# agentmorris/MegaDetector

Hardware: AMD Instinct MI355X
Metric: images/sec (whole node) MDv5a @1280px batch inference (higher is better)
Workload: dtype bf16

## Files before the change

megadetector_amd/csrc/conv_v2.cpp:

```cpp

#include <algorithm>
#include <type_traits>

#include "conv_device.h"

namespace mdhip {
namespace MDHIP_ST {

namespace {

constexpr int v2_lds_bytes(int bm, int bn) { return 2 * (bm + bn) * 128; }
constexpr int v2_ring_lds_bytes(int bm, int bn) { return (3 * bm + 2 * bn) * 128; }
constexpr int v2_blocks_per_cu(int bm, int bn, int nw) {
    int b = 163840 / v2_lds_bytes(bm, bn);
    if (b > 32 / nw) b = 32 / nw;
    if (b > 2) b = 2;
    return b < 1 ? 1 : b;
}
constexpr int v2_waves_per_simd(int bm, int bn, int nw) {
    int w = v2_blocks_per_cu(bm, bn, nw) * nw / 4;
    return w < 1 ? 1 : w;
}

}

template <int BM, int BN, int WM, int WN, int PROF = 0, bool UP = false, int PW = 0, int RA = 2, int DEC = 0>
__global__ void __launch_bounds__(WM * WN * 64, v2_waves_per_simd(BM, BN, WM * WN))
conv_v2_kernel(const ConvArgs p) {
#if defined(__HIP_DEVICE_COMPILE__)
    constexpr int NW = WM * WN;
    constexpr int TM = BM / WM, TN = BN / WN;
    constexpr int FM = TM / 16, FN = TN / 16;
    constexpr int A_BYTES = BM * 128, B_BYTES = BN * 128, STAGE = A_BYTES + B_BYTES;
    constexpr int B_INSTR = BN / 8;
    constexpr int A_PER = BM / 8 / NW, B_PER = (B_INSTR + NW - 1) / NW;
    constexpr bool B_RAGGED = (B_INSTR % NW) != 0;
    static_assert((BM / 8) % NW == 0, "the activation tile must split evenly over the waves");
    static_assert(RA == 2 || (RA == 3 && PW != 0 && !UP), "the three-stage activation ring is a pointwise instantiation");
    auto a_stage = [](int sa) __attribute__((always_inline)) { return RA == 2 ? sa * STAGE : sa * A_BYTES; };
    auto b_stage = [](int sb) __attribute__((always_inline)) { return RA == 2 ? sb * STAGE + A_BYTES : RA * A_BYTES + sb * B_BYTES; };
    static_assert(TM % 16 == 0 && TN % 16 == 0 && TM % 8 == 0, "wave tile must be a multiple of 16x16");

    extern __shared__ __attribute__((aligned(16))) char smem_generic[];
    lds_char* const smem = (lds_char*)smem_generic;

    const int tid = threadIdx.x;
    const int lane = tid & 63;
    const int wave = __builtin_amdgcn_readfirstlane(tid >> 6);
    const int wm = wave / WN, wn = wave % WN;

    const int xcd = blockIdx.x & 7, slot = blockIdx.x >> 3;
    const int tile_n = slot % p.tiles_n;
    const int ms = slot / p.tiles_n;
    const int xcd_first = xcd * p.tiles_per_xcd;
    const int xcd_tiles = min(p.tiles_per_xcd, p.tiles_m - xcd_first);
    const int my_tiles = (xcd_tiles > ms) ? (xcd_tiles - ms + p.m_streams - 1) / p.m_streams : 0;
    if (my_tiles <= 0) return;
    const int first_tile = xcd_first + ms;
    const int tile_step = p.m_streams;
    const int last_tile = first_tile + (my_tiles - 1) * tile_step;
    const int n0 = tile_n * BN;
    const int KT = p.k_pad >> 6;
    const int total_steps = my_tiles * KT;

    const int lr = lane >> 3;
    const int jj = (lane & 7) ^ lr;
    const __amdgpu_buffer_rsrc_t b_rsrc = __builtin_amdgcn_make_buffer_rsrc(
        (void*)(p.wgt + (size_t)n0 * p.k_pad), 0, kNumRecords, kRsrcFlags);
    unsigned b_off[B_PER];
#pragma unroll
    for (int i = 0; i < B_PER; ++i) {
        const int row = (i * NW + wave) * 8 + lr;
        b_off[i] = (n0 + row < p.n_rows) ? (unsigned)(row * p.k_pad + jj * 8) * 2u : kOOB;
    }

    __amdgpu_buffer_rsrc_t a_rsrc = b_rsrc;
    unsigned a_off[A_PER];
    uint32_t a_mask[A_PER];
    const int up_slabs = UP ? p.up_slabs : 0;
    [[maybe_unused]] const __amdgpu_buffer_rsrc_t u_rsrc = __builtin_amdgcn_make_buffer_rsrc((void*)(UP ? p.in_up : p.in), 0, kNumRecords, kRsrcFlags);
    [[maybe_unused]] unsigned u_off[UP ? A_PER : 1];
    int c8 = 0, ts = 0;
    uint32_t tapbit = 1;
    unsigned tapoff = 0;
    int l_kt = 0, l_tile = first_tile;
    bool l_live = true;
    [[maybe_unused]] int lb_kt = 0;
    const int kh = p.ntaps / p.kw;
    const unsigned wrap_c = (unsigned)(p.ld_in * 2 - p.C8 * 16);
    const unsigned wrap_r = (unsigned)((p.W - p.kw) * p.ld_in * 2);

    auto init_tile = [&](int tile_m) __attribute__((always_inline)) {
        if constexpr (PW) {
            const int m0 = tile_m * BM;
            const long long left = ((long long)p.M - m0) * p.ld_in * 2;
            a_rsrc = __builtin_amdgcn_make_buffer_rsrc((void*)(p.in + (long long)m0 * p.ld_in), 0,
                                                       (int)(left > 0x7fffffffLL ? 0x7fffffffLL : left), kRsrcFlags);
#pragma unroll
            for (int i = 0; i < A_PER; ++i) {
                const int row = (i * NW + wave) * 8 + lr;
                a_off[i] = (unsigned)(row * p.ld_in * 2 + jj * 16);
                a_mask[i] = 1u;
            }
            c8 = jj; ts = 0; tapbit = 1; tapoff = 0;
            return;
        }
        const int m0 = tile_m * BM;
        const int b0 = conv_udiv(m0, p.HoWo, p.rcp_howo);
        const int rem0 = m0 - b0 * p.HoWo;
        const int oy0 = conv_udiv(rem0, p.Wo, p.rcp_wo);
        const int ox0 = rem0 - oy0 * p.Wo;
        const long long base_px = (long long)(b0 * p.H + oy0 * p.stride - p.pad) * p.W + (ox0 * p.stride - p.pad);
        a_rsrc = __builtin_amdgcn_make_buffer_rsrc((void*)(p.in + base_px * p.ld_in), 0, kNumRecords, kRsrcFlags);
#pragma unroll
        for (int i = 0; i < A_PER; ++i) {
            const int row = (i * NW + wave) * 8 + lr;
            const int m = m0 + row;
            uint32_t mask = 0;
            unsigned off = 0;
            if (m < p.M) {
                const int b = conv_udiv(m, p.HoWo, p.rcp_howo);
                const int rem = m - b * p.HoWo;
                const int oy = conv_udiv(rem, p.Wo, p.rcp_wo);
                const int ox = rem - oy * p.Wo;
                const int iy0 = oy * p.stride - p.pad;
                const int ix0 = ox * p.stride - p.pad;
                const long long px = (long long)(b * p.H + iy0) * p.W + ix0;
                off = (unsigned)((px - base_px) * p.ld_in * 2);
                if constexpr (UP)
                    u_off[i] = (unsigned)((((long long)b * (p.H >> 1) + (oy >> 1)) * (p.W >> 1) + (ox >> 1)) * p.ld_up * 2 + jj * 16);
                uint32_t cols = 0, rows = 0;
#pragma unroll
                for (int t = 0; t < 3; ++t) {
                    cols |= (t < p.kw && (unsigned)(ix0 + t) < (unsigned)p.W) ? 1u << t : 0u;
                    rows |= (t < kh && (unsigned)(iy0 + t) < (unsigned)p.H) ? 1u << t : 0u;
                }
                mask = ((rows & 1u) ? cols : 0u) | ((rows & 2u) ? cols << p.kw : 0u) | ((rows & 4u) ? cols << (2 * p.kw) : 0u);
            }
            a_off[i] = off;
            a_mask[i] = mask;
        }
        c8 = jj; ts = 0; tapbit = 1; tapoff = (unsigned)jj * 16u;
    };

    [[maybe_unused]] const bool pw_tail_bad = (p.C8 & 7) != 0 && jj >= (p.C8 & 7);
    auto advance = [&]() __attribute__((always_inline)) {
        if (++l_kt == KT) {
            l_kt = 0;
            if (l_tile == last_tile) {
                l_live = false;
#pragma unroll
                for (int i = 0; i < A_PER; ++i) a_mask[i] = 0;
            } else {
                l_tile += tile_step;
                init_tile(l_tile);
            }
        } else {
            if constexpr (PW) {
                if constexpr (PW == 2) {
                    if (l_kt == KT - 1 && pw_tail_bad) {
#pragma unroll
                        for (int i = 0; i < A_PER; ++i) a_off[i] = kOOB;
                    }
                }
            }
            c8 += 8;
            tapoff += 128u;
            const bool w = c8 >= p.C8;
            c8 = w ? c8 - p.C8 : c8;
            tapoff += w ? wrap_c : 0u;
            tapbit = w ? tapbit << 1 : tapbit;
            ts += w ? 1 : 0;
            const bool w2 = ts == p.kw;
            ts = w2 ? 0 : ts;
            tapoff += w2 ? wrap_r : 0u;
        }
    };

    auto dma_a = [&](int buf, int i) __attribute__((always_inline)) {
        if constexpr ((PROF & 16) != 0) return;
        if constexpr (UP) {
            if (l_kt < up_slabs) {
                MDHIP_DMA16(u_rsrc, smem + buf * STAGE + (i * NW + wave) * 1024, (a_mask[i] & tapbit) ? u_off[i] : kOOB, l_kt * 128);
                return;
            }
        }
        if constexpr (PW) {
            MDHIP_DMA16(a_rsrc, smem + a_stage(buf) + (i * NW + wave) * 1024, a_off[i], l_kt * 128);
        } else {
            const unsigned voff = (a_mask[i] & tapbit) ? a_off[i] + tapoff : kOOB;
            MDHIP_DMA16(a_rsrc, smem + buf * STAGE + (i * NW + wave) * 1024, voff, 0);
        }
    };
    auto dma_b = [&](int buf, int i) __attribute__((always_inline)) {
        if constexpr ((PROF & 16) != 0) return;
        if (B_RAGGED && i == B_PER - 1 && wave >= B_INSTR % NW) return;
        const unsigned voff = (PW || l_live) ? b_off[i] : kOOB;
        MDHIP_DMA16(b_rsrc, smem + b_stage(buf) + (i * NW + wave) * 1024, voff, (RA == 3 ? lb_kt : l_kt) * 128);
    };

    const int frag_row_off = (lane & 15) * 128;
    const int frag_ch0 = (((lane >> 4) ^ (lane & 7)) * 16);
    const int a_frag_base = (wm * TM) * 128 + frag_row_off;
    const int b_frag_base = (wn * TN) * 128 + frag_row_off;
    auto read_x = [&](int buf, int kk, int i) -> frag8_t {
        if constexpr ((PROF & 32) != 0) return frag_dummy(lane + i);
        return *(const __attribute__((address_space(3))) frag8_t*)(smem + a_stage(buf) + a_frag_base + i * 2048 +
                                                                 (frag_ch0 ^ (kk * 64)));
    };
    auto read_w = [&](int buf, int kk, int j) -> frag8_t {
        if constexpr ((PROF & 32) != 0) return frag_dummy(lane + j);
        return *(const __attribute__((address_space(3))) frag8_t*)(smem + b_stage(buf) + b_frag_base + j * 2048 +
                                                                 (frag_ch0 ^ (kk * 64)));
    };

    f32x4 acc[FM][FN];
#pragma unroll
    for (int i = 0; i < FM; ++i)
#pragma unroll
        for (int j = 0; j < FN; ++j) acc[i][j] = f32x4{0.f, 0.f, 0.f, 0.f};

    const int q4 = lane >> 4;
    auto epilogue_t = [&](int tile_m, auto has_res_t, auto out_f32_t, auto out_f8_t) {
#pragma clang fp contract(off)
        constexpr bool HAS_RES = decltype(has_res_t)::value;
        constexpr bool OUT_F32 = decltype(out_f32_t)::value;
        constexpr bool OUT_F8 = decltype(out_f8_t)::value;
        const int m0 = tile_m * BM + wm * TM + (lane & 15);
        const int nbase = n0 + wn * TN + q4 * 4;
        int lane_e = lane;
        asm volatile("" : "+v"(lane_e));
        float neg_log2e = kNegLog2e;
        asm volatile("" : "+v"(neg_log2e));
        const int ml = wm * TM + (lane_e & 15);
        const int qe = lane_e >> 4;
        const int npair0 = n0 + wn * TN + qe * 8;
        const int nlast = n0 + wn * TN + (FN - 1) * 16 + qe * 4;
        const long long rows_left = (long long)p.M - (long long)tile_m * BM;
        const __amdgpu_buffer_rsrc_t o_rsrc = __builtin_amdgcn_make_buffer_rsrc(
            (void*)((uint16_t*)p.out + (size_t)tile_m * BM * p.ld_out), 0,
            (OUT_F32 || OUT_F8) ? 0 : (int)min(rows_left * p.ld_out * 2, 0x7fffffffLL), kRsrcFlags);
        const unsigned o_pair = ((unsigned)ml * (unsigned)p.ld_out + (unsigned)npair0) * 2u;
        const unsigned o_last = ((unsigned)ml * (unsigned)p.ld_out + (unsigned)nlast) * 2u;
        const unsigned o_step = 16u * (unsigned)p.ld_out * 2u;
        const __amdgpu_buffer_rsrc_t r_rsrc = __builtin_amdgcn_make_buffer_rsrc(
            (void*)(p.res + (HAS_RES ? (size_t)tile_m * BM * p.ld_res : 0)), 0,
            HAS_RES ? (int)min(rows_left * p.ld_res * 2, 0x7fffffffLL) : 0, kRsrcFlags);
        const unsigned r_col = ((unsigned)ml * (unsigned)p.ld_res + (unsigned)(n0 + wn * TN + qe * 4)) * 2u;
        const unsigned r_step = 16u * (unsigned)p.ld_res * 2u;
        float bv[FN][4];
#pragma unroll
        for (int j = 0; j < FN; ++j) {
            const int nb = n0 + wn * TN + j * 16;
            bv[j][0] = bv[j][1] = bv[j][2] = bv[j][3] = 0.f;
            if (nb < p.n_rows) {
                f32x16 b16;
                const unsigned long long ba = (unsigned long long)(p.bias + nb);
                const unsigned long long bs =
                    ((unsigned long long)(unsigned)__builtin_amdgcn_readfirstlane((int)(ba >> 32)) << 32) |
                    (unsigned)__builtin_amdgcn_readfirstlane((int)ba);
                asm volatile("s_load_dwordx16 %0, %1, 0x0\n\ts_waitcnt lgkmcnt(0)" : "=s"(b16) : "s"(bs) : "memory");
                const f32x4 g0 = {b16[0], b16[1], b16[2], b16[3]}, g1 = {b16[4], b16[5], b16[6], b16[7]},
                            g2 = {b16[8], b16[9], b16[10], b16[11]}, g3 = {b16[12], b16[13], b16[14], b16[15]};
                const f32x4 g = q4 == 0 ? g0 : (q4 == 1 ? g1 : (q4 == 2 ? g2 : g3));
                bv[j][0] = g[0]; bv[j][1] = g[1]; bv[j][2] = g[2]; bv[j][3] = g[3];
            }
        }
        uint2 rrow[2][FN];
        auto fetch_res_row = [&](int i, uint2 (&r)[FN]) {
#pragma unroll
            for (int j = 0; j < FN; ++j) {
                const u32x2 t = __builtin_amdgcn_raw_buffer_load_b64(r_rsrc, (int)(r_col + (unsigned)i * r_step + (unsigned)(j * 32)), 0, 0);
                r[j] = make_uint2(t[0], t[1]);
            }
        };
        if constexpr (HAS_RES) fetch_res_row(0, rrow[0]);
#pragma unroll
        for (int i = 0; i < FM; ++i) {
            if constexpr (HAS_RES) {
                if (i + 1 < FM) fetch_res_row(i + 1, rrow[(i + 1) & 1]);
            }
            const int m = m0 + i * 16;
            float v[FN][4];
#pragma unroll
            for (int j = 0; j < FN; ++j) {
#pragma unroll
                for (int r = 0; r < 4; r += 2) {
                    const mdhip_f32x2 t = mdhip_f32x2{acc[i][j][r], acc[i][j][r + 1]} + mdhip_f32x2{bv[j][r], bv[j][r + 1]};
                    v[j][r] = t[0];
                    v[j][r + 1] = t[1];
                }
                acc[i][j] = f32x4{0.f, 0.f, 0.f, 0.f};
            }
            if ((PROF & 4) == 0 && p.act) {
#pragma unroll
                for (int j = 0; j < FN; ++j) {
#pragma unroll
                    for (int r = 0; r < 4; r += 2) {
                        const mdhip_f32x2 t = silu_f32x2(mdhip_f32x2{v[j][r], v[j][r + 1]}, neg_log2e);
                        v[j][r] = t[0];
                        v[j][r + 1] = t[1];
                    }
                }
            }
#pragma unroll
            for (int j = 0; j < FN; ++j) {
                if constexpr (HAS_RES) {
                    const uint2 rv = rrow[i & 1][j];
                    v[j][0] += st_unpack((uint16_t)(rv.x & 0xffff));
                    v[j][1] += st_unpack((uint16_t)(rv.x >> 16));
                    v[j][2] += st_unpack((uint16_t)(rv.y & 0xffff));
                    v[j][3] += st_unpack((uint16_t)(rv.y >> 16));
                }
            }
            if constexpr ((PROF & 2) != 0) {
#pragma unroll
                for (int j = 0; j < FN; ++j) asm volatile("" ::"v"(v[j][0]), "v"(v[j][1]), "v"(v[j][2]), "v"(v[j][3]));
            } else if constexpr (OUT_F32 && DEC != 0) {
#pragma unroll
                for (int j = 0; j < FN; ++j) {
                    const int n = nbase + j * 16;
                    if (m < p.M && n < p.N) mdhip_decode_store(p, m, n, v[j]);
                }
            } else if constexpr (OUT_F32) {
#pragma unroll
                for (int j = 0; j < FN; ++j) {
                    const int n = nbase + j * 16;
                    if (m < p.M && n < p.N)
                        *(float4*)((float*)p.out + (size_t)m * p.ld_out + n) = make_float4(v[j][0], v[j][1], v[j][2], v[j][3]);
                }
            } else if constexpr (OUT_F8) {
                const __amdgpu_buffer_rsrc_t o8_rsrc = __builtin_amdgcn_make_buffer_rsrc(
                    (void*)((uint8_t*)p.out + (size_t)tile_m * BM * p.ld_out), 0, (int)min(rows_left * p.ld_out, 0x7fffffffLL), kRsrcFlags);
                const unsigned row8 = (unsigned)(ml + i * 16) * (unsigned)p.ld_out;
#pragma unroll
                for (int j = 0; j + 1 < FN; j += 2) {
                    const unsigned a0 = pack_e4m3x4(v[j][0], v[j][1], v[j][2], v[j][3], p.out_qscale);
                    const unsigned b0 = pack_e4m3x4(v[j + 1][0], v[j + 1][1], v[j + 1][2], v[j + 1][3], p.out_qscale);
                    const auto s0 = __builtin_amdgcn_permlane32_swap(a0, b0, false, false);
                    const auto t0 = __builtin_amdgcn_permlane16_swap(s0[0], s0[1], false, false);
                    const int n = npair0 + j * 16;
                    __builtin_amdgcn_raw_buffer_store_b64(u32x2{t0[0], t0[1]}, o8_rsrc, (int)(n < p.N ? row8 + (unsigned)n : kOOB), 0, 0);
                }
                if (FN & 1) {
                    const int j = FN - 1;
                    __builtin_amdgcn_raw_buffer_store_b32(pack_e4m3x4(v[j][0], v[j][1], v[j][2], v[j][3], p.out_qscale), o8_rsrc,
                                                          (int)(nlast < p.N ? row8 + (unsigned)nlast : kOOB), 0, 0);
                }
            } else {
#pragma unroll
                for (int j = 0; j + 1 < FN; j += 2) {
                    unsigned a0 = st_pack2(v[j][0], v[j][1]), a1 = st_pack2(v[j][2], v[j][3]);
                    unsigned b0 = st_pack2(v[j + 1][0], v[j + 1][1]), b1 = st_pack2(v[j + 1][2], v[j + 1][3]);
                    auto s0 = __builtin_amdgcn_permlane32_swap(a0, b0, false, false);
                    auto s1 = __builtin_amdgcn_permlane32_swap(a1, b1, false, false);
                    auto t0 = __builtin_amdgcn_permlane16_swap(s0[0], s0[1], false, false);
                    auto t1 = __builtin_amdgcn_permlane16_swap(s1[0], s1[1], false, false);
                    const unsigned off = o_pair + (unsigned)i * o_step + (unsigned)(j * 32);
                    __builtin_amdgcn_raw_buffer_store_b128(u32x4{t0[0], t1[0], t0[1], t1[1]}, o_rsrc,
                                                           (int)(npair0 + j * 16 < p.N ? off : kOOB), 0, 0);
                }
                if (FN & 1) {
                    const int j = FN - 1;
                    __builtin_amdgcn_raw_buffer_store_b64(u32x2{st_pack2(v[j][0], v[j][1]), st_pack2(v[j][2], v[j][3])}, o_rsrc,
                                                          (int)(nlast < p.N ? o_last + (unsigned)i * o_step : kOOB), 0, 0);
                }
            }
        }
    };
    auto epilogue = [&](int tile_m) {
        if constexpr ((PROF & 8) != 0) __builtin_amdgcn_s_setprio(3);
        if constexpr (DEC != 0) { epilogue_t(tile_m, std::false_type{}, std::true_type{}, std::false_type{}); return; }
        if (p.out_f32) epilogue_t(tile_m, std::false_type{}, std::true_type{}, std::false_type{});
        else if (p.out_f8) epilogue_t(tile_m, std::false_type{}, std::false_type{}, std::true_type{});
        else if (p.res) epilogue_t(tile_m, std::true_type{}, std::false_type{}, std::false_type{});
        else epilogue_t(tile_m, std::false_type{}, std::false_type{}, std::false_type{});
        if constexpr ((PROF & 8) != 0) __builtin_amdgcn_s_setprio(0);
    };

    init_tile(first_tile);
    auto lb_advance = [&]() __attribute__((always_inline)) { lb_kt = (lb_kt + 1 == KT) ? 0 : lb_kt + 1; };
    if constexpr (RA == 3) {
#pragma unroll
        for (int st = 0; st < 3; ++st) {
#pragma unroll
            for (int i = 0; i < A_PER; ++i) dma_a(st, i);
            advance();
        }
#pragma unroll
        for (int st = 0; st < 2; ++st) {
#pragma unroll
            for (int i = 0; i < B_PER; ++i) dma_b(st, i);
            lb_advance();
        }
    } else {
#pragma unroll
        for (int i = 0; i < A_PER; ++i) dma_a(0, i);
#pragma unroll
        for (int i = 0; i < B_PER; ++i) dma_b(0, i);
        advance();
#pragma unroll
        for (int i = 0; i < A_PER; ++i) dma_a(1, i);
#pragma unroll
        for (int i = 0; i < B_PER; ++i) dma_b(1, i);
        advance();
    }
    asm volatile("s_waitcnt vmcnt(0)" ::: "memory");
    __builtin_amdgcn_s_barrier();
    frag8_t xa[FM], wa[FN], xb[FM], wb[FN];
#pragma unroll
    for (int i = 0; i < FM; ++i) xa[i] = read_x(0, 0, i);
#pragma unroll
    for (int j = 0; j < FN; ++j) wa[j] = read_w(0, 0, j);

    int c_kt = 0, c_tile = first_tile;
    unsigned long long t_acc[6] = {0, 0, 0, 0, 0, 0}, t_prev = 0;
    auto stamp = [&](int k) {
        if constexpr ((PROF & 1) != 0) {
            const unsigned long long t = __builtin_amdgcn_s_memtime();
            t_acc[k] += t - t_prev;
            t_prev = t;
        }
    };
    if constexpr ((PROF & 1) != 0) t_prev = __builtin_amdgcn_s_memtime();
    [[maybe_unused]] int ca = 0;
    for (int step = 0; step < total_steps; ++step) {
        const int cur = step & 1;
        const int xa_cur = RA == 3 ? ca : cur, xa_nxt = RA == 3 ? (ca == 2 ? 0 : ca + 1) : cur ^ 1;
        constexpr int DMA_TOTAL = A_PER + B_PER, DMA_PER_G = (DMA_TOTAL + FN - 1) / FN;
#pragma unroll
        for (int g = 0; g < FN; ++g) {
            wb[g] = read_w(cur, 1, g);
            if (g < FM) xb[g] = read_x(xa_cur, 1, g);
            if (g == FN - 1) {
#pragma unroll
                for (int i = FN; i < FM; ++i) xb[i] = read_x(xa_cur, 1, i);
            }
            __builtin_amdgcn_sched_barrier(0);
            if constexpr ((PROF & 64) == 0) {
#pragma unroll
                for (int i = 0; i < FM; ++i)
                    acc[i][g] = MDHIP_MFMA(wa[g], xa[i], acc[i][g]);
            }
            __builtin_amdgcn_sched_barrier(0);
        }

        stamp(0);
        if constexpr (RA == 3) asm volatile("s_waitcnt vmcnt(%0) lgkmcnt(0)" ::"n"(A_PER) : "memory");
        else asm volatile("s_waitcnt vmcnt(0) lgkmcnt(0)" ::: "memory");
        stamp(1);
        __builtin_amdgcn_s_barrier();
        stamp(2);
        __builtin_amdgcn_sched_barrier(0);

#pragma unroll
        for (int g = 0; g < FN; ++g) {
            wa[g] = read_w(cur ^ 1, 0, g);
            if (g < FM) xa[g] = read_x(xa_nxt, 0, g);
            if (g == FN - 1) {
#pragma unroll
                for (int i = FN; i < FM; ++i) xa[i] = read_x(xa_nxt, 0, i);
            }
            __builtin_amdgcn_sched_barrier(0);
            if constexpr ((PROF & 64) == 0) {
#pragma unroll
                for (int i = 0; i < FM; ++i)
                    acc[i][g] = MDHIP_MFMA(wb[g], xb[i], acc[i][g]);
            }
            __builtin_amdgcn_sched_barrier(0);
#pragma unroll
            for (int d = g * DMA_PER_G; d < (g + 1) * DMA_PER_G && d < DMA_TOTAL; ++d) {
                if constexpr (RA == 3) {
                    if (d < B_PER) dma_b(cur, d);
                    else dma_a(xa_cur, d - B_PER);
                } else {
                    if (d < A_PER) dma_a(cur, d);
                    else dma_b(cur, d - A_PER);
                }
            }
            __builtin_amdgcn_sched_barrier(0);
        }

        stamp(3);
        advance();
        if constexpr (RA == 3) {
            lb_advance();
            ca = ca == 2 ? 0 : ca + 1;
        }
        stamp(4);
        if (++c_kt == KT) {
            epilogue(c_tile);
            c_kt = 0;
            c_tile += tile_step;
        }
        stamp(5);
    }
    if constexpr ((PROF & 1) != 0) {
        if (lane == 0 && p.dbg) {
            unsigned long long* d = (unsigned long long*)p.dbg + ((size_t)blockIdx.x * NW + wave) * 8;
            for (int k = 0; k < 6; ++k) d[k] = t_acc[k];
            d[6] = (unsigned long long)total_steps;
            d[7] = (unsigned long long)__builtin_amdgcn_s_getreg(((4 - 1) << 11) | (0 << 6) | 20) ;
        }
    }
#endif
}

#include "conv_v2_stream.h"

#define MDHIP_CONV2_CFGS(X) \
    X(0, 160, 160, 2, 2)    \
    X(1, 128, 160, 2, 2)    \
    X(2, 160, 80, 2, 1)     \
    X(3, 128, 80, 4, 1)     \
    X(4, 96, 160, 2, 2)     \
    X(5, 64, 160, 1, 2)     \
    X(6, 192, 160, 4, 2)    \
    X(7, 256, 160, 4, 2)    \
    X(8, 320, 160, 4, 2)
#define MDHIP_CONV2_RING(X) \
    X(9, 96, 160, 2, 2)     \
    X(10, 64, 160, 1, 2)    \
    X(11, 320, 160, 4, 2)   \
    X(12, 256, 160, 4, 2)
#define MDHIP_CONV2_DEC(X) \
    X(0, 160, 160, 2, 2)   \
    X(2, 160, 80, 2, 1)    \
    X(3, 128, 80, 4, 1)    \
    X(8, 320, 160, 4, 2)
#define MDHIP_CONV2_PROF(X) \
    X(13, 160, 160, 2, 2, 1)  \
    X(14, 320, 160, 4, 2, 1) \
    X(15, 160, 160, 2, 2, 54) \
    X(16, 320, 160, 4, 2, 22) \
    X(17, 320, 160, 4, 2, 16) \
    X(18, 160, 160, 2, 2, 16)
#define MDHIP_CONV2_PROFRING(X) \
    X(19, 320, 160, 4, 2, 1)  \
    X(20, 320, 160, 4, 2, 2)  \
    X(21, 320, 160, 4, 2, 16) \
    X(22, 320, 160, 4, 2, 64)

static const ConvCfg g_cfgs2[] = {
#define X(id, bm, bn, wm, wn)                                                                        \
    {bm, bn, (wm) * (wn) * 64, (size_t)v2_lds_bytes(bm, bn), v2_blocks_per_cu(bm, bn, (wm) * (wn)), \
     "v2:" #bm "x" #bn "/" #wm "x" #wn},
    MDHIP_CONV2_CFGS(X)
#undef X
#define X(id, bm, bn, wm, wn)                                                                        \
    {bm, bn, (wm) * (wn) * 64, (size_t)v2_ring_lds_bytes(bm, bn), 163840 / v2_ring_lds_bytes(bm, bn) >= 2 ? 2 : 1, "v2:" #bm "x" #bn "/" #wm "x" #wn "/a3"},
    MDHIP_CONV2_RING(X)
#undef X
#define X(id, bm, bn, wm, wn, prof)                                                                  \
    {bm, bn, (wm) * (wn) * 64, (size_t)v2_lds_bytes(bm, bn), v2_blocks_per_cu(bm, bn, (wm) * (wn)), \
     "v2prof" #prof ":" #bm "x" #bn "/" #wm "x" #wn},
    MDHIP_CONV2_PROF(X)
#undef X
#define X(id, bm, bn, wm, wn, prof)                                                                  \
    {bm, bn, (wm) * (wn) * 64, (size_t)v2_ring_lds_bytes(bm, bn), 1, "v2prof" #prof ":" #bm "x" #bn "/" #wm "x" #wn "/a3"},
    MDHIP_CONV2_PROFRING(X)
#undef X
};
constexpr int kNumPlain2 = 0 MDHIP_CONV2_CFGS(MDHIP_COUNT_ROW);
constexpr int kNumCfgs2 = kNumPlain2 MDHIP_CONV2_RING(MDHIP_COUNT_ROW);
constexpr int kNumProf = 0 MDHIP_CONV2_PROF(MDHIP_COUNT_ROW) MDHIP_CONV2_PROFRING(MDHIP_COUNT_ROW);

namespace {
enum { V2_PLAIN = 0, V2_PW1, V2_PW2, V2_UP, V2_DEV, V2_DEV_PW, V2_STREAM };
constexpr int kStreamMinM = 307200;
ConvInstTable conv2_insts() {
    static const ConvInst t[] = {
#define X(id, bm, bn, wm, wn)                                                                                         \
    MDHIP_INST(id, V2_PLAIN, (wm) * (wn) * 64, v2_lds_bytes(bm, bn), conv_v2_kernel<bm, bn, wm, wn>)                  \
    MDHIP_INST(id, V2_PW1, (wm) * (wn) * 64, v2_lds_bytes(bm, bn), conv_v2_kernel<bm, bn, wm, wn, 0, false, 1>)       \
    MDHIP_INST(id, V2_PW2, (wm) * (wn) * 64, v2_lds_bytes(bm, bn), conv_v2_kernel<bm, bn, wm, wn, 0, false, 2>)
        MDHIP_CONV2_CFGS(X)
#undef X
#define X(id, bm, bn, wm, wn)                                                                                         \
    MDHIP_INST(id, V2_PW1, (wm) * (wn) * 64, v2_ring_lds_bytes(bm, bn), conv_v2_kernel<bm, bn, wm, wn, 0, false, 1, 3>) \
    MDHIP_INST(id, V2_PW2, (wm) * (wn) * 64, v2_ring_lds_bytes(bm, bn), conv_v2_kernel<bm, bn, wm, wn, 0, false, 2, 3>)
        MDHIP_CONV2_RING(X)
#undef X
#define X(id, bm, bn, wm, wn, prof) MDHIP_INST(id, V2_DEV, (wm) * (wn) * 64, v2_lds_bytes(bm, bn), conv_v2_kernel<bm, bn, wm, wn, prof>)
        MDHIP_CONV2_PROF(X)
#undef X
#define X(id, bm, bn, wm, wn, prof) MDHIP_INST(id, V2_DEV_PW, (wm) * (wn) * 64, v2_ring_lds_bytes(bm, bn), conv_v2_kernel<bm, bn, wm, wn, prof, false, 1, 3>)
        MDHIP_CONV2_PROFRING(X)
#undef X
#define X(id, bm, bn, wm, wn) MDHIP_INST(id, CONV_KEY_DEC, (wm) * (wn) * 64, v2_lds_bytes(bm, bn), conv_v2_kernel<bm, bn, wm, wn, 0, false, 1, 2, 1>)
        MDHIP_CONV2_DEC(X)
#undef X
        MDHIP_INST(0, V2_UP, 256, v2_lds_bytes(160, 160), conv_v2_kernel<160, 160, 2, 2, 0, true>)
        MDHIP_INST(0, V2_STREAM, 256, 0, conv_v2_stream_kernel)
    };
    return {t, (int)(sizeof(t) / sizeof(t[0]))};
}
bool conv2_streams(const ConvArgs& a, bool pw) {
    if (a.pw_stream <= 0 || (a.pw_stream == 1 && a.M < kStreamMinM) || !pw || a.k_pad != 192 || a.C8 != 20 || a.n_rows != 160 || a.N != 160 ||
        a.act != 1 || a.out_f32 || a.res || a.in_up || a.in_f8 || a.out_f8 || a.dec_pred || a.M <= 0 || (a.ld_in % 8) != 0 ||
        (a.ld_out % 8) != 0 || a.ld_in < 160 || a.ld_out < 160 || ((uintptr_t)a.in % 16) != 0 || ((uintptr_t)a.out % 16) != 0)
        return false;
    const long long in0 = (long long)(uintptr_t)a.in, out0 = (long long)(uintptr_t)a.out;
    const long long in1 = in0 + ((long long)(a.M - 1) * a.ld_in + 160) * 2, out1 = out0 + ((long long)(a.M - 1) * a.ld_out + 160) * 2;
    if (in1 <= out0 || out1 <= in0) return true;
    if (a.ld_in != a.ld_out) return false;
    const long long pitch = (long long)a.ld_in * 2, r = (((out0 - in0) % pitch) + pitch) % pitch;
    return r >= 320 && r + 320 <= pitch;
}
const ConvInst* conv2_pick(int cfg, const ConvArgs& a) {
    const ConvInstTable t = conv2_insts();
    if (a.in_up) return a.dec_pred ? nullptr : conv_find_inst(t, cfg, V2_UP);
    const bool pw = a.ntaps == 1 && a.stride == 1 && a.pad == 0 && a.H == a.Ho && a.W == a.Wo, whole = (a.C8 & 7) == 0;
    if (a.dec_pred) return pw && whole && a.out_f32 ? conv_find_inst(t, cfg, CONV_KEY_DEC) : nullptr;
    if (cfg >= kNumCfgs2) {
        const ConvInst* dev = conv_find_inst(t, cfg, V2_DEV);
        return dev || !(pw && whole) ? dev : conv_find_inst(t, cfg, V2_DEV_PW);
    }
    if (cfg >= 0 && conv2_streams(a, pw)) return conv_find_inst(t, 0, V2_STREAM);
    return conv_find_inst(t, cfg, !pw ? V2_PLAIN : whole ? V2_PW1 : V2_PW2);
}

bool conv2_cfg_is_ring(int cfg) { return cfg >= kNumPlain2 && cfg < kNumCfgs2; }
bool conv2_shape_ok(const ConvArgs& a) {
    if (a.in_up && !(a.ntaps == 1 && a.stride == 1 && (a.H % 2) == 0 && (a.W % 2) == 0 && a.up_slabs > 0 &&
                     a.up_slabs * 8 <= a.C8 && !a.in_f8))
        return false;
    return a.C8 >= 8 && a.kw <= 3 && a.ntaps <= 9 && (a.k_pad % 64) == 0;
}
bool conv2_supports(int cfg, const ConvArgs& a) {
    if (cfg < 0 || cfg >= kNumCfgs2 + kNumProf) return false;
    if (conv2_cfg_is_ring(cfg) && a.k_pad < 3 * 64) return false;
    return conv2_shape_ok(a) && conv2_pick(cfg, a) != nullptr;
}

hipError_t conv2_launch(int cfg, const ConvArgs& a, hipStream_t s) {
    if (cfg < 0 || cfg >= kNumCfgs2 + kNumProf || !conv2_shape_ok(a)) return hipErrorInvalidValue;
    ConvArgs p = a;
    conv_set_rcp(p);
    dim3 grid = conv_tile_grid(p, g_cfgs2[cfg]);
    const ConvInst* inst = conv2_pick(cfg, a);
    if (inst && inst->key == V2_STREAM) {
        const int streams = std::max(1, std::min(1024, (p.M + 15) / 16 / 2));
        grid = dim3((unsigned)((streams + 3) / 4));
    }
    return conv_launch_inst(inst, grid, p, s);
}
int conv2_variant(int cfg, const ConvArgs& a) {
    if (cfg < 0 || cfg >= kNumCfgs2 + kNumProf || !conv2_shape_ok(a)) return -1;
    const ConvInst* inst = conv2_pick(cfg, a);
    return inst ? inst->key : -1;
}
}

MDHIP_CONV_FAMILY(conv_v2, CONV_V2, g_cfgs2, kNumCfgs2, kNumProf, true, false, true, conv2_supports, conv2_launch, conv2_insts, conv2_variant)

}
}
```

Baseline: 1111.

## Add persistent streaming kernel for 320-channel pointwise convolutions

Adds a persistent streaming kernel for 1x1 convolutions with 320 input and 320 output channels plus SiLU. Each block keeps its slice of the weights in registers and streams row tiles of the activations through a multi-slot LDS ring with async buffer loads. The kernel replaces the tiled GEMM path for these layers when M is large. The aim is to overlap memory traffic with MFMA work and avoid reloading weights for every tile. The cost is heavy register use at one block per CU and a narrow shape guard that sends every other layer to the old path.

Measured after the change: 1114 (median of 5 runs). About the same (+0.2%).

```diff
diff --git a/megadetector_amd/csrc/conv_v2.cpp b/megadetector_amd/csrc/conv_v2.cpp
--- a/megadetector_amd/csrc/conv_v2.cpp
+++ b/megadetector_amd/csrc/conv_v2.cpp
@@ -507,6 +507,7 @@
 }
 
 #include "conv_v2_stream.h"
+#include "conv_v2_stream320.h"
 
 #define MDHIP_CONV2_CFGS(X) \
     X(0, 160, 160, 2, 2)    \
@@ -566,8 +567,19 @@
 constexpr int kNumProf = 0 MDHIP_CONV2_PROF(MDHIP_COUNT_ROW) MDHIP_CONV2_PROFRING(MDHIP_COUNT_ROW);
 
 namespace {
-enum { V2_PLAIN = 0, V2_PW1, V2_PW2, V2_UP, V2_DEV, V2_DEV_PW, V2_STREAM };
+enum { V2_PLAIN = 0, V2_PW1, V2_PW2, V2_UP, V2_DEV, V2_DEV_PW, V2_STREAM, V2_STREAM320 };
 constexpr int kStreamMinM = 307200;
+#define MDHIP_CONV2_STREAM320(X) \
+    X(0, 4, 3, true)             \
+    X(1, 2, 4, true)             \
+    X(2, 2, 4, false)
+constexpr int kStream320U[] = {
+#define X(id, u, r, ov) u,
+    MDHIP_CONV2_STREAM320(X)
+#undef X
+};
+constexpr int kNumStream320 = (int)(sizeof(kStream320U) / sizeof(kStream320U[0]));
+constexpr int kStream320MinM = 409600;
 ConvInstTable conv2_insts() {
     static const ConvInst t[] = {
 #define X(id, bm, bn, wm, wn)                                                                                         \
@@ -592,6 +604,9 @@
 #undef X
         MDHIP_INST(0, V2_UP, 256, v2_lds_bytes(160, 160), conv_v2_kernel<160, 160, 2, 2, 0, true>)
         MDHIP_INST(0, V2_STREAM, 256, 0, conv_v2_stream_kernel)
+#define X(id, u, r, ov) MDHIP_INST(id, V2_STREAM320, 256, (r) * (u) * 10240, conv_v2_stream320_kernel<u, r, ov>)
+        MDHIP_CONV2_STREAM320(X)
+#undef X
     };
     return {t, (int)(sizeof(t) / sizeof(t[0]))};
 }
@@ -607,6 +622,18 @@
     const long long pitch = (long long)a.ld_in * 2, r = (((out0 - in0) % pitch) + pitch) % pitch;
     return r >= 320 && r + 320 <= pitch;
 }
+bool conv2_streams320(const ConvArgs& a, bool pw) {
+    if (a.pw_stream <= 0 || (a.pw_stream == 1 && a.M < kStream320MinM) || !pw || a.k_pad != 320 || a.C8 != 40 || a.n_rows != 320 || a.N != 320 ||
+        a.act != 1 || a.out_f32 || a.res || a.in_up || a.in_f8 || a.out_f8 || a.dec_pred || a.M <= 0 || (a.ld_in % 8) != 0 ||
+        (a.ld_out % 8) != 0 || a.ld_in < 320 || a.ld_out < 320 || ((uintptr_t)a.in % 16) != 0 || ((uintptr_t)a.out % 16) != 0)
+        return false;
+    const long long in0 = (long long)(uintptr_t)a.in, out0 = (long long)(uintptr_t)a.out;
+    const long long in1 = in0 + ((long long)(a.M - 1) * a.ld_in + 320) * 2, out1 = out0 + ((long long)(a.M - 1) * a.ld_out + 320) * 2;
+    if (in1 <= out0 || out1 <= in0) return true;
+    if (a.ld_in != a.ld_out) return false;
+    const long long pitch = (long long)a.ld_in * 2, r = (((out0 - in0) % pitch) + pitch) % pitch;
+    return r >= 640 && r + 640 <= pitch;
+}
 const ConvInst* conv2_pick(int cfg, const ConvArgs& a) {
     const ConvInstTable t = conv2_insts();
     if (a.in_up) return a.dec_pred ? nullptr : conv_find_inst(t, cfg, V2_UP);
@@ -617,6 +644,7 @@
         return dev || !(pw && whole) ? dev : conv_find_inst(t, cfg, V2_DEV_PW);
     }
     if (cfg >= 0 && conv2_streams(a, pw)) return conv_find_inst(t, 0, V2_STREAM);
+    if (cfg >= 0 && conv2_streams320(a, pw)) return conv_find_inst(t, a.dev_param > 0 && a.dev_param < kNumStream320 ? a.dev_param : 0, V2_STREAM320);
     return conv_find_inst(t, cfg, !pw ? V2_PLAIN : whole ? V2_PW1 : V2_PW2);
 }
 
@@ -643,6 +671,10 @@
         const int streams = std::max(1, std::min(1024, (p.M + 15) / 16 / 2));
         grid = dim3((unsigned)((streams + 3) / 4));
     }
+    if (inst && inst->key == V2_STREAM320) {
+        const int rows = 16 * kStream320U[inst->local], units = (p.M + rows - 1) / rows;
+        grid = dim3((unsigned)std::max(1, std::min(256, units / 2)));
+    }
     return conv_launch_inst(inst, grid, p, s);
 }
 int conv2_variant(int cfg, const ConvArgs& a) {
diff --git a/megadetector_amd/csrc/conv_v2_stream320.h b/megadetector_amd/csrc/conv_v2_stream320.h
--- /dev/null
+++ b/megadetector_amd/csrc/conv_v2_stream320.h
@@ -0,0 +1,138 @@
+#pragma once
+
+template <int N>
+__device__ __forceinline__ void stream320_wait() {
+    asm volatile("s_waitcnt vmcnt(%0) lgkmcnt(0)" ::"n"(N) : "memory");
+}
+template <int K, int KMAX, int BASE, int STEP>
+__device__ __forceinline__ void stream320_wait_unit(int t) {
+    if constexpr (K >= KMAX) {
+        stream320_wait<BASE + STEP * KMAX>();
+    } else {
+        if (t == K) stream320_wait<BASE + STEP * K>();
+        else stream320_wait_unit<K + 1, KMAX, BASE, STEP>(t);
+    }
+}
+
+template <int U, int R, bool OV>
+__global__ void __launch_bounds__(256, 1)
+conv_v2_stream320_kernel(const ConvArgs p) {
+#if defined(__HIP_DEVICE_COMPILE__)
+    constexpr int NC = 5;
+    constexpr int KS = 10;
+    constexpr int ROWS = 16 * U;
+    constexpr int SLAB = ROWS * 128, SLOT = 5 * SLAB;
+    constexpr int PIECES = 2 * U;
+    constexpr int P = 5 * PIECES / 4;
+    constexpr int S = 3 * U;
+    static_assert(U >= 2 && U % 2 == 0, "the pieces of a unit split evenly over the four waves");
+    static_assert(R >= 2 && R * SLOT <= 163840, "the ring fits the CU's LDS");
+    static_assert((R - 2) * (P + S) <= 63, "vmcnt is a 6-bit counter");
+
+    extern __shared__ __attribute__((aligned(16))) char smem_generic[];
+    lds_char* const smem = (lds_char*)smem_generic;
+
+    const int lane = threadIdx.x & 63;
+    const int wave = __builtin_amdgcn_readfirstlane(threadIdx.x >> 6);
+    const int px = lane & 15, q = lane >> 4;
+    const int n_grid = (int)gridDim.x;
+    const int n_units = (p.M + ROWS - 1) / ROWS;
+    const int iters = ((int)blockIdx.x < n_units) ? (n_units - (int)blockIdx.x + n_grid - 1) / n_grid : 0;
+
+    const __amdgpu_buffer_rsrc_t w_rsrc = __builtin_amdgcn_make_buffer_rsrc((void*)p.wgt, 0, p.n_rows * p.k_pad * 2, kRsrcFlags);
+    const __amdgpu_buffer_rsrc_t b_rsrc = __builtin_amdgcn_make_buffer_rsrc((void*)p.bias, 0, p.n_rows * 4, kRsrcFlags);
+    const int n0 = wave * (NC * 16);
+    frag8_t w[NC][KS];
+    f32x4 bv[NC];
+#pragma unroll
+    for (int j = 0; j < NC; ++j) {
+        const unsigned row = (unsigned)((n0 + j * 16 + px) * p.k_pad + q * 8) * 2u;
+#pragma unroll
+        for (int s = 0; s < KS; ++s)
+            w[j][s] = __builtin_bit_cast(frag8_t, __builtin_amdgcn_raw_buffer_load_b128(w_rsrc, (int)row + s * 64, 0, 0));
+        bv[j] = __builtin_bit_cast(f32x4, __builtin_amdgcn_raw_buffer_load_b128(b_rsrc, (n0 + j * 16 + q * 4) * 4, 0, 0));
+    }
+    __builtin_amdgcn_s_waitcnt(0x0f70);
+    MDHIP_FENCE();
+
+    auto unit_of = [&](int it) __attribute__((always_inline)) { return it * n_grid + (int)blockIdx.x; };
+    auto rows_rsrc = [&](const void* base, int ld, int unit) __attribute__((always_inline)) {
+        const long long left = ((long long)p.M - (long long)unit * ROWS) * ld * 2;
+        return __builtin_amdgcn_make_buffer_rsrc((void*)((const uint16_t*)base + (long long)unit * ROWS * ld), 0,
+                                                 (int)(left <= 0 ? 0LL : left > 0x7fffffffLL ? 0x7fffffffLL : left), kRsrcFlags);
+    };
+    const int lr = lane >> 3, jj = (lane & 7) ^ lr;
+    unsigned x_off[PIECES / 4];
+#pragma unroll
+    for (int g = 0; g < PIECES / 4; ++g) x_off[g] = (unsigned)(((g * 4 + wave) * 8 + lr) * p.ld_in * 2 + jj * 16);
+    auto dma = [&](int slot, int it) __attribute__((always_inline)) {
+        const __amdgpu_buffer_rsrc_t r = rows_rsrc(p.in, p.ld_in, unit_of(it));
+        lds_char* const dst = smem + slot * SLOT + wave * 1024;
+#pragma unroll
+        for (int i = 0; i < P; ++i) {
+            const int slab = (i * 4) / PIECES, first = (i * 4) % PIECES;
+            MDHIP_DMA16(r, dst + slab * SLAB + first * 1024, x_off[first / 4], slab * 128);
+        }
+    };
+    const int frag_a = px * 128 + ((q ^ (lane & 7)) * 16);
+    const int frag_b = frag_a ^ 64;
+    const unsigned o_pair = (unsigned)(px * p.ld_out + n0 + q * 8) * 2u;
+    const unsigned o_last = (unsigned)(px * p.ld_out + n0 + (NC - 1) * 16 + q * 4) * 2u;
+    const int o_step = 16 * p.ld_out * 2;
+    auto compute = [&](int slot, int it) __attribute__((always_inline)) {
+#pragma clang fp contract(off)
+        const lds_char* const src = smem + slot * SLOT;
+        const __amdgpu_buffer_rsrc_t o_rsrc = rows_rsrc(p.out, p.ld_out, unit_of(it));
+        frag8_t x[KS];
+        auto read_group = [&](int g) __attribute__((always_inline)) {
+#pragma unroll
+            for (int s = 0; s < KS; ++s)
+                x[s] = *(const __attribute__((address_space(3))) frag8_t*)(src + (s >> 1) * SLAB + g * 2048 + ((s & 1) ? frag_b : frag_a));
+        };
+        read_group(0);
+#pragma unroll
+        for (int g = 0; g < U; ++g) {
+            if (!OV || g == 0) MDHIP_FENCE();
+            f32x4 acc[NC];
+#pragma unroll
+            for (int j = 0; j < NC; ++j) acc[j] = f32x4{0.f, 0.f, 0.f, 0.f};
+#pragma unroll
+            for (int s = 0; s < KS; ++s)
+#pragma unroll
+                for (int j = 0; j < NC; ++j) acc[j] = MDHIP_MFMA(w[j][s], x[s], acc[j]);
+            MDHIP_FENCE();
+            if (g + 1 < U) read_group(g + 1);
+            MDHIP_FENCE();
+            float v[NC][4];
+#pragma unroll
+            for (int j = 0; j < NC; ++j) {
+                mdhip_bias4(acc[j], bv[j], v[j]);
+                mdhip_silu4(v[j]);
+            }
+#pragma unroll
+            for (int j = 0; j + 1 < NC; j += 2)
+                __builtin_amdgcn_raw_buffer_store_b128(conv_pack_pair(v[j], v[j + 1]), o_rsrc, (int)(o_pair + (unsigned)(g * o_step + j * 32)), 0, 0);
+            __builtin_amdgcn_raw_buffer_store_b64(u32x2{st_pack2(v[NC - 1][0], v[NC - 1][1]), st_pack2(v[NC - 1][2], v[NC - 1][3])}, o_rsrc,
+                                                  (int)(o_last + (unsigned)(g * o_step)), 0, 0);
+        }
+    };
+#pragma unroll
+    for (int d = 0; d < R - 1; ++d) {
+        dma(d, d);
+        MDHIP_FENCE();
+    }
+    int cs = 0, ls = R - 1;
+    for (int it = 0; it < iters; ++it) {
+        stream320_wait_unit<0, R - 2, (R - 2) * P, S>(it);
+        __builtin_amdgcn_s_barrier();
+        MDHIP_FENCE();
+        dma(ls, it + R - 1);
+        MDHIP_FENCE();
+        compute(cs, it);
+        MDHIP_FENCE();
+        cs = cs + 1 == R ? 0 : cs + 1;
+        ls = ls + 1 == R ? 0 : ls + 1;
+    }
+    asm volatile("s_waitcnt vmcnt(0)" ::: "memory");
+#endif
+}
```
